# goroda/GPEXP

Measured on AMD Instinct MI355X. Metric: GP-fit+IVAR-eval points/s at N=32768 d=8 (wall-time in ms_per_step); value = (N+M)/t_step, SURVEY 8d's N/t_fit and M/t_IVAR are points_per_s_fit / points_per_s_ivar right behind it, higher is better.
Workload: dtype f64; 1 GPU; C4: N=32768 d=8 Matern-5/2 (rho=0.5,s=1,noise=0.1) kfill+potrf+potrs+logdet+IVAR over M=32768 MC points; N=32768, d=8, M=32768, kernel=matern52, seed=32768, parallelism=1 GPU

## Files before the change

gpexp_amd/_lib.py:

```python
import ctypes as C
import os

import numpy as np

_HERE = os.path.dirname(os.path.abspath(__file__))
LIB_PATH = os.path.join(_HERE, "libgpx_hip.so")

c_i64 = C.c_int64
c_dp = C.POINTER(C.c_double)
c_ip = C.POINTER(c_i64)
c_vp = C.c_void_p

_SIGS = {
    "gpx_abi_version": (C.c_int, []),
    "gpx_last_error": (C.c_char_p, []),
    "gpx_create": (C.c_int, [C.c_int, C.POINTER(c_vp)]),
    "gpx_destroy": (C.c_int, [c_vp]),
    "gpx_sync": (C.c_int, [c_vp]),
    "gpx_trim": (C.c_int, [c_vp]),
    "gpx_device_info": (C.c_int, [c_vp, C.c_char_p, C.c_int, C.POINTER(C.c_int), c_ip, C.POINTER(C.c_int)]),
    "gpx_mat_from_host": (C.c_int, [c_vp, c_dp, c_i64, c_i64, C.c_int, C.POINTER(c_vp)]),
    "gpx_mat_alloc": (C.c_int, [c_vp, c_i64, c_i64, C.c_int, C.POINTER(c_vp)]),
    "gpx_mat_free": (C.c_int, [c_vp, c_vp]),
    "gpx_mat_clone": (C.c_int, [c_vp, c_vp, C.POINTER(c_vp)]),
# ... 106 lines not shown
    "gpx_graph_free": (C.c_int, [c_vp, c_vp]),
    "gpx_dist2_unpack_rows": (C.c_int, [c_vp, c_vp, c_i64, c_i64, c_i64, c_i64, c_vp, c_i64, c_i64, c_i64]),
    "gpx_dist2_unpack_diag": (C.c_int, [c_vp, c_vp, c_i64, c_i64, c_i64, c_vp, c_i64]),
    "gpx_dist2_unpack_diag_at": (C.c_int, [c_vp, c_vp, c_i64, c_i64, c_i64, c_vp, c_i64, c_i64]),
    "gpx_dist2_trsv_diag": (C.c_int, [c_vp, c_vp, c_i64, c_i64, c_i64, c_vp, c_i64, C.c_int]),
    "gpx_dist2_gemv": (C.c_int, [c_vp, c_vp, c_i64, c_i64, c_i64, c_i64, c_vp, c_i64, c_vp, c_i64, C.c_int]),
    "gpx_dist2_logdet_acc": (C.c_int, [c_vp, c_vp, c_i64, c_i64, c_i64, c_i64, c_vp]),
    "gpx_stream_select": (C.c_int, [c_vp, C.c_int]),
    "gpx_event_record": (C.c_int, [c_vp, C.c_int]),
    "gpx_event_wait": (C.c_int, [c_vp, C.c_int]),
    "gpx_dist_finish": (C.c_int, [c_vp, c_vp]),
    "gpx_ivar_grad": (C.c_int, [c_vp, C.c_int, C.c_int, c_dp, C.c_int, c_vp, c_vp, c_vp, c_dp, c_dp]),
    "gpx_ivar_grad_w": (C.c_int, [c_vp, C.c_int, C.c_int, c_dp, C.c_int, c_vp, c_vp, c_vp, c_dp, c_vp, c_dp]),
    "gpx_ivar_grad_rows": (C.c_int, [c_vp, C.c_int, C.c_int, c_dp, C.c_int, c_vp, c_vp, c_vp, c_vp, c_i64, c_dp]),
    "gpx_var_grad": (C.c_int, [c_vp, C.c_int, C.c_int, c_dp, C.c_int, c_vp, c_vp, c_vp, c_dp, c_dp, c_dp, c_dp]),
    "gpx_var_grad_newpt": (C.c_int, [c_vp, C.c_int, C.c_int, c_dp, C.c_int, c_vp, c_vp, c_vp, c_dp]),
    "gpx_fitc_var_grad": (C.c_int, [c_vp, c_vp, C.c_int, C.c_int, c_dp, C.c_int, c_vp, c_vp, c_dp, c_dp, c_dp, c_dp]),
    "gpx_fitc_var_grad_newpt": (C.c_int, [c_vp, c_vp, C.c_int, C.c_int, c_dp, C.c_int, c_vp, c_vp, c_dp]),
    "gpx_profile_enable": (C.c_int, [c_vp, C.c_int]),
    "gpx_profile_reset": (C.c_int, [c_vp]),
    "gpx_profile_get": (C.c_int, [c_vp, C.c_int, c_ip, c_dp, c_dp, c_dp]),
    "gpx_dbg_gemm": (C.c_int, [c_vp, c_vp, c_vp, c_vp, C.c_int, C.c_int, C.c_int]),
    "gpx_dbg_gemm_strassen": (C.c_int, [c_vp, c_vp, c_vp, c_vp]),
    "gpx_dbg_gemm_tri": (C.c_int, [c_vp, c_vp, c_vp, c_vp, C.c_int, C.c_int, C.c_int]),
    "gpx_dbg_gemm_ksplit": (C.c_int, [c_vp, c_vp, c_vp, c_vp, C.c_int, C.c_int]),
    "gpx_dbg_kfill_plan": (C.c_int, [c_vp, C.c_int, C.c_int, c_dp, C.c_int, c_vp, c_vp, C.POINTER(C.c_int), c_dp]),
    "gpx_dbg_colreduce_plan": (C.c_int, [c_i64, c_i64, C.POINTER(c_i64), C.POINTER(c_i64)]),
    "gpx_dbg_panel_bcast_plan": (C.c_int, [C.c_int, C.c_int, c_i64, C.c_int, C.POINTER(c_i64), C.POINTER(C.c_int),
                                           C.POINTER(c_i64), c_i64, C.POINTER(c_i64)]),
    "gpx_dbg_guard_violations": (c_i64, [c_vp]),
    "gpx_dbg_guard_selftest": (C.c_int, [c_vp]),
    "gpx_dbg_spin": (C.c_int, [c_vp, C.c_int]),
    "gpx_dbg_spin_us": (C.c_int, [c_vp, c_i64]),
    "gpx_dbg_stamp": (C.c_int, [c_vp, C.c_int]),
    "gpx_dbg_spin_until": (C.c_int, [c_vp, C.c_int, c_i64]),
    "gpx_dbg_event_elapsed": (C.c_int, [c_vp, C.c_int, C.c_int, c_dp]),
    "gpx_dbg_leaf_stamps": (C.c_int, [c_vp, c_vp, C.c_int, C.POINTER(c_i64)]),
}

_lib = None


def load():
    global _lib
    if _lib is not None:
        return _lib
# ... 51 lines not shown
```

gpexp_amd/csrc/api.hip:

```cpp
#include "gpx_internal.h"
#include <stdarg.h>
#include <stdio.h>
#include <string.h>
#include <math.h>
#include <stdlib.h>

static thread_local char g_err[1024] = "";

void gpx_set_error(const char* fmt, ...) {
  va_list ap;
  va_start(ap, fmt);
  vsnprintf(g_err, sizeof(g_err), fmt, ap);
  va_end(ap);
}

static constexpr int64_t GUARD = 4096;

int gpx_dev_alloc(gpx_ctx* ctx, int64_t bytes, void** out) {
  if (bytes <= 0) bytes = 8;
  bytes = gpx_round_up(bytes, 256);
  const int64_t key = bytes + (ctx->guard ? 2 * GUARD : 0);
  void* base = nullptr;
  auto it = ctx->pool.find(key);
  if (it != ctx->pool.end()) {
// ... 1397 lines not shown
  GPX_TRY(gpx_dev_alloc(ctx, pb, &P));
  int r = mode <= 1 ? launch_gemm_ksplit(ctx, A->p, A->ld, B->p, B->ld, C->p, C->ld, m, n, k, mode == 1, parts, (double*)P)
                    : launch_gemm_ksplit_small(ctx, A->p, A->ld, B->p, B->ld, C->p, C->ld, m, n, k, mode == 3, parts, (double*)P);
  (void)hipStreamSynchronize(ctx->stream);
  gpx_dev_release(ctx, P, pb);
  return r;
}

int gpx_dbg_gemm(gpx_ctx* ctx, const gpx_mat* A, const gpx_mat* B, gpx_mat* C, int bt, int accumulate, int lower) {
  GPX_ARG(ctx && A && B && C, "NULL argument");
  const int64_t m = C->prows, n = C->pcols, k = A->pcols;
  GPX_ARG(A->prows == m, "A rows");
  GPX_ARG(bt ? (B->prows == n && B->pcols == k) : (B->prows == k && B->pcols == n), "B shape");
  GPX_TRY(launch_gemm(ctx, A->p, A->ld, B->p, B->ld, C->p, C->ld, m, n, k, bt != 0, accumulate != 0,
                      lower != 0));
  GPX_HIP(hipStreamSynchronize(ctx->stream));
  return 0;
}

int gpx_dbg_gemm_strassen(gpx_ctx* ctx, const gpx_mat* A, const gpx_mat* B, gpx_mat* C) {
  GPX_ARG(ctx && A && B && C, "NULL argument");
  const int64_t m = C->prows, n = C->pcols, k = A->pcols;
  GPX_ARG(A->prows == m && B->prows == k && B->pcols == n, "operand shapes");
  GPX_TRY(launch_gemm_strassen(ctx, A->p, A->ld, B->p, B->ld, C->p, C->ld, m, n, k, nullptr, 0));
  GPX_HIP(hipStreamSynchronize(ctx->stream));
  return 0;
}

}
```

gpexp_amd/csrc/chol.hip:

```cpp
#include "gpx_internal.h"
#include <math.h>
#include <stdlib.h>
#include <stddef.h>

namespace {

constexpr int NB = GPX_TILE;
constexpr int LS = NB + 1;

typedef double d4 __attribute__((ext_vector_type(4)));

__device__ __forceinline__ double readlane_d(double v, int srclane) {
  int lo = __builtin_amdgcn_readlane(__double2loint(v), srclane);
  int hi = __builtin_amdgcn_readlane(__double2hiint(v), srclane);
  return __hiloint2double(hi, lo);
}

constexpr int LB = 16;
constexpr int TS17 = LB + 1;
constexpr int BSZ = LB * TS17;
constexpr int LEAF_CB = LB * LB + 64 + LB;

__device__ __forceinline__ constexpr int sb_off(int I, int J) { return (I * (I + 1) / 2 + J) * BSZ; }

// ... 1176 lines not shown
  if (!Lm->binv) {
    void* p;
    GPX_TRY(gpx_dev_alloc(ctx, bytes, &p));
    Lm->binv = (double*)p;
    Lm->binv_bytes = bytes;
  }
  void* pt;
  GPX_TRY(gpx_dev_alloc(ctx, nblk * ib * ib * 8, &pt));
  int r = binv_build_range(ctx, Lm->p, Lm->ld, Lm->aux, Lm->binv, ib, n, (double*)pt);
  if (r == 0) r = chol_binv_finish(ctx, Lm, ib);
  (void)hipStreamSynchronize(ctx->stream);
  gpx_dev_release(ctx, pt, nblk * ib * ib * 8);
  if (r != 0) Lm->binv_ib = 0;
  return r;
}

struct PotrsPlan {
  const double* L;
  int64_t ld, n, ib, nblk;
  int64_t sib;
  const double* binv;
  const double* binvT;
  double* part;
  bool strassen = false;
  double* sscr = nullptr;
  int64_t sscr_bytes = 0;
};
static inline int64_t blk_off(const PotrsPlan& P, int64_t b) { return b * P.ib < P.n ? b * P.ib : P.n; }
static inline const double* blk_inv(const PotrsPlan& P, const double* base, int64_t b) {
  const int64_t row = b * P.ib, sb = row / P.sib, within = row - sb * P.sib;
  return base + sb * P.sib * P.sib + within * P.sib + within;
}

static int potrs_fwd(gpx_ctx* ctx, const PotrsPlan& P, int64_t b0, int64_t b1, double* rhs, double* x) {
  if (b1 - b0 == 1) {
    const int64_t o = blk_off(P, b0), sz = blk_off(P, b0 + 1) - o;
    hipLaunchKernelGGL(binv_gemv_kernel, dim3((unsigned)((sz + 3) / 4)), dim3(256), 0, ctx->stream, blk_inv(P, P.binv, b0),
                       P.sib, sz, rhs + o, x + o, 1);
    return 0;
  }
  const int64_t mid = (b0 + b1) / 2;
  GPX_TRY(potrs_fwd(ctx, P, b0, mid, rhs, x));
  const int64_t r0 = blk_off(P, mid), r1 = blk_off(P, b1), c0 = blk_off(P, b0);
  int64_t wg = (r1 - r0 + 3) / 4;
  if (wg > 4096) wg = 4096;
  hipLaunchKernelGGL(gemv_sub_kernel, dim3((unsigned)wg), dim3(256), 0, ctx->stream, P.L + r0 * P.ld + c0, P.ld, r1 - r0, r0 - c0,
                     x + c0, rhs + r0);
  return potrs_fwd(ctx, P, mid, b1, rhs, x);
}

static int potrs_bwd(gpx_ctx* ctx, const PotrsPlan& P, int64_t b0, int64_t b1, double* rhs, double* z) {
  if (b1 - b0 == 1) {
    const int64_t o = blk_off(P, b0), sz = blk_off(P, b0 + 1) - o;
    hipLaunchKernelGGL(binv_gemv_kernel, dim3((unsigned)((sz + 3) / 4)), dim3(256), 0, ctx->stream, blk_inv(P, P.binvT, b0),
                       P.sib, sz, rhs + o, z + o, 0);
    return 0;
  }
  const int64_t mid = (b0 + b1) / 2;
  GPX_TRY(potrs_bwd(ctx, P, mid, b1, rhs, z));
  const int64_t r0 = blk_off(P, mid), r1 = blk_off(P, b1), c0 = blk_off(P, b0);
  GPX_TRY(launch_colreduce(ctx, P.L + r0 * P.ld + c0, P.ld, r1 - r0, r0 - c0, z + r0, rhs + c0, P.part, 1));
  return potrs_bwd(ctx, P, b0, mid, rhs, z);
}

#ifndef GPX_STRASSEN_MIN_ROWS
#define GPX_STRASSEN_MIN_ROWS 8192
#endif
#ifndef GPX_STRASSEN_MIN_COLS
#define GPX_STRASSEN_MIN_COLS 4096
#endif
static inline bool strassen_gate(int64_t rows, int64_t cols, int64_t k) {
  return rows >= GPX_STRASSEN_MIN_ROWS && k >= GPX_STRASSEN_MIN_ROWS && cols >= GPX_STRASSEN_MIN_COLS &&
         gemm_strassen_scratch_bytes(rows, cols, k) > 0;
}

static int trsm_left_oop_rec(gpx_ctx* ctx, const PotrsPlan& P, int64_t b0, int64_t b1, double* B, int64_t ldb, double* W,
                             int64_t ldw, int64_t m) {
  if (b1 - b0 == 1) {
    const int64_t o = blk_off(P, b0), sz = blk_off(P, b0 + 1) - o;
    return launch_gemm_tri(ctx, blk_inv(P, P.binv, b0), P.sib, B + o * ldb, ldb, W + o * ldw, ldw, sz, m, sz, false, false,
                           false, 1);
  }
  const int64_t mid = (b0 + b1) / 2;
  GPX_TRY(trsm_left_oop_rec(ctx, P, b0, mid, B, ldb, W, ldw, m));
  const int64_t r0 = blk_off(P, mid), r1 = blk_off(P, b1), c0 = blk_off(P, b0);
  if (P.strassen && strassen_gate(r1 - r0, m, r0 - c0))
    GPX_TRY(launch_gemm_strassen(ctx, P.L + r0 * P.ld + c0, P.ld, W + c0 * ldw, ldw, B + r0 * ldb, ldb, r1 - r0, m, r0 - c0,
                                 P.sscr, P.sscr_bytes));
  else
    GPX_TRY(launch_gemm(ctx, P.L + r0 * P.ld + c0, P.ld, W + c0 * ldw, ldw, B + r0 * ldb, ldb, r1 - r0, m, r0 - c0, false,
                        true, false));
  return trsm_left_oop_rec(ctx, P, mid, b1, B, ldb, W, ldw, m);
}

int chol_trsm_left_oop(gpx_ctx* ctx, gpx_mat* Lm, double* B, int64_t ldb, double* W, int64_t ldw, int64_t m) {
  GPX_ARG(Lm && Lm->factored && Lm->aux && B && W && B != W, "trsm: matrix has not been factored / bad buffers");
  if (m == 0) return 0;
  GPX_TRY(chol_binv_ensure(ctx, Lm));
  PotrsPlan P;
  P.L = Lm->p;
  P.ld = Lm->ld;
  P.n = Lm->prows;
  P.sib = Lm->binv_ib;
  P.ib = P.sib < 1024 ? P.sib : 1024;
  P.nblk = (P.n + P.ib - 1) / P.ib;
  P.binv = Lm->binv;
  P.binvT = nullptr;
  P.part = nullptr;
  void* ps = nullptr;
  int64_t sbytes = 0;
  if (P.nblk >= 2 && env_i64("GPX_STRASSEN", 1) != 0) {
    const int64_t r0 = blk_off(P, P.nblk / 2);
    if (strassen_gate(P.n - r0, m, r0)) {
      sbytes = gemm_strassen_scratch_bytes(P.n - r0, m, r0);
      if (gpx_dev_alloc(ctx, sbytes, &ps) != 0) {
        (void)hipGetLastError();
        ps = nullptr;
      }
    }
  }
  P.strassen = ps != nullptr;
  P.sscr = (double*)ps;
  P.sscr_bytes = sbytes;
  const int r = trsm_left_oop_rec(ctx, P, 0, P.nblk, B, ldb, W, ldw, m);
  if (ps) {
    (void)hipStreamSynchronize(ctx->stream);
    gpx_dev_release(ctx, ps, sbytes);
  }
  return r;
}

int chol_trsm_left_group(gpx_ctx* ctx, const double* Lg, int64_t ld, const double* invd, int64_t w, int64_t below, int64_t ib,
                         double* B, int64_t ldb, int64_t m, double* inv, double* tmp, double* W, int64_t ldw) {
  GPX_ARG(Lg && invd && B && inv && tmp && W && W != B && w > 0 && w % NB == 0 && ib >= NB && ib % NB == 0, "trsm group: bad arguments");
  if (m == 0) return 0;
  GPX_TRY(binv_build_range(ctx, Lg, ld, invd, inv, ib, w, tmp));
  PotrsPlan P;
  P.L = Lg;
  P.ld = ld;
  P.n = w;
  P.ib = P.sib = ib;
  P.nblk = (w + ib - 1) / ib;
  P.binv = inv;
  P.binvT = nullptr;
// ... 71 lines not shown
```

gpexp_amd/csrc/gemm_f64.hip:

```cpp
#include "gpx_internal.h"
#include <stdlib.h>

namespace {

typedef double d4 __attribute__((ext_vector_type(4)));

constexpr int KB = 16;
constexpr int SA = KB + 1;

template <bool BT, int TE>
struct Smem {
  double a[2][TE * SA];
  double b[2][BT ? TE * SA : KB * (TE + 16)];
};

template <bool LOWER>
__device__ __forceinline__ bool tile_of(int sblk, int within, int tiles_m, int tiles_n, int sb_cols, int sb_shift,
                                        int* by, int* bx, int rot = 0) {
  const int sbm = (1 << sb_shift) - 1;
  int sr, sc;
  if (LOWER) {
    const int nsr = (tiles_m + sbm) >> sb_shift;
    const int noff = nsr * (nsr - 1) / 2;
    if (sblk < noff) {
// ... 19 lines not shown
  if (!LOWER && rot == 2) {
    *by = (sr << sb_shift) + (within & sbm);
    *bx = (sc << sb_shift) + (sbm - (within >> sb_shift));
  }
  if (!LOWER && rot == 4) {
    *by = (sr << sb_shift) + (sbm - (within >> sb_shift));
    *bx = (sc << sb_shift) + (within & sbm);
  }
  if (!LOWER && rot == 3) {
    *by = (sr << sb_shift) + (within & sbm);
    *bx = (sc << sb_shift) + (within >> sb_shift);
  }
  if (*by >= tiles_m || *bx >= tiles_n) return false;
  if (LOWER && *bx > *by) return false;
  return true;
}

struct NoSeg {
  static constexpr bool on = false;
};

struct NoDual {
  static constexpr bool on = false;
};
struct Dual {
  static constexpr bool on = true;
  double* c2;
  double s;
};

template <bool BT, bool ACC, int TE, class SEGF = NoSeg, class EPI = NoDual>
__device__ __forceinline__ void gemm_tile(Smem<BT, TE>& sm, const double* A, int64_t lda, const double* B, int64_t ldb,
                                          double* C, int64_t ldc, int nk, int by, int bx, const SEGF& segf = SEGF(),
                                          const EPI& epi = EPI()) {
  constexpr int SBN = TE + 16;
  constexpr int FI = TE / 32;
  constexpr int NL = TE / 32;
  constexpr int WS = TE / 2;
  constexpr int BKR = 512 / TE;
  constexpr int A_BUF = TE * SA;
  constexpr int B_BUF = BT ? TE * SA : KB * SBN;

  const int t = threadIdx.x;
  const int lane = t & 63, wave = t >> 6;
  const int wm = wave >> 1, wn = wave & 1;
  const int64_t m0 = (int64_t)by * TE, n0 = (int64_t)bx * TE;

  const int ar = t >> 3, ac = (t & 7) * 2;
  const int br = t / (TE / 2), bc = (t % (TE / 2)) * 2;
  const unsigned voff_a = (unsigned)((ar * lda + ac) * 8);
  const unsigned voff_b = BT ? (unsigned)((ar * ldb + ac) * 8) : (unsigned)((br * ldb + bc) * 8);
// ... 166 lines not shown
      GPX_MFMAS(3);
      GPX_FRAGS(buf ^ 1, 3, 3);
    }
    }
    GPX_MFMAS(0);
    GPX_MFMAS(1);
    GPX_MFMAS(2);
    GPX_MFMAS(3);
#undef GPX_STEP
#undef GPX_FRAGS
#undef GPX_MFMAS
#undef GPX_PIN
#undef GPX_PIN_ALL
  }
#undef GPX_GLOAD
#undef GPX_GLOAD_AT
#undef GPX_LD16
#undef GPX_SSTORE
#undef GPX_ST2
#undef GPX_STB
#undef GPX_COMPUTE

  double* Cw = C + (m0 + wm * WS + fk) * ldc + n0 + wn * WS + fr;
  if constexpr (EPI::on) {
    static_assert(ACC, "the two-destination epilogue accumulates");
    double* Cw2 = epi.c2 + (m0 + wm * WS + fk) * ldc + n0 + wn * WS + fr;
    const double s2 = epi.s;
#pragma unroll
    for (int i = 0; i < FI; ++i)
#pragma unroll
      for (int v = 0; v < 4; ++v) {
        double* cp = Cw + (int64_t)(i * 16 + 4 * v) * ldc;
        double* cq = Cw2 + (int64_t)(i * 16 + 4 * v) * ldc;
        double cv[FI], cw[FI];
#pragma unroll
        for (int j = 0; j < FI; ++j) {
          cv[j] = cp[j * 16];
          cw[j] = cq[j * 16];
        }
#pragma unroll
        for (int j = 0; j < FI; ++j) {
          cp[j * 16] = cv[j] - acc[i][j][v];
          cq[j * 16] = cw[j] - s2 * acc[i][j][v];
        }
      }
    return;
  }
// ... 49 lines not shown
    B += k0;
    nkt = nk - by * (TE / KB);
  }
  if (tri == 4) {
    const int64_t k0 = (int64_t)bx * TE;
    A += k0;
    B += k0 * ldb;
    nkt = nk - bx * (TE / KB);
  }
  gemm_tile<BT, ACC, TE>(sm, A, lda, B, ldb, C, ldc, nkt, by, bx);
}

template <int TE>
__global__ __launch_bounds__(256, 2) void gemm_f64_dual_kernel(const double* A, int64_t lda, const double* B, int64_t ldb,
                                                               double* C, double* C2, double s, int64_t ldc, int nk,
                                                               int tiles_m, int tiles_n, int sb_cols, int sb_shift) {
  __shared__ Smem<false, TE> sm;
  const int w = blockIdx.x;
  const int xcd = w & 7, q = w >> 3;
  const int sbs2 = 2 * sb_shift;
  int by, bx;
  if (!tile_of<false>((q >> sbs2) * 8 + xcd, q & ((1 << sbs2) - 1), tiles_m, tiles_n, sb_cols, sb_shift, &by, &bx, 0)) return;
  gemm_tile<false, true, TE, NoSeg, Dual>(sm, A, lda, B, ldb, C, ldc, nk, by, bx, NoSeg(), Dual{C2, s});
}

template <bool BSIDE>
__global__ __launch_bounds__(256) void strassen_sums_kernel(const double* __restrict__ X, int64_t ldx, int64_t hr, int64_t hc,
                                                            double* __restrict__ S, int64_t lds, int64_t sstride) {
  const int64_t j = ((int64_t)blockIdx.x * 256 + threadIdx.x) * 2;
  if (j >= hc) return;
  for (int64_t i = blockIdx.y; i < hr; i += gridDim.y) {
    const double* x1 = X + i * ldx + j;
    const double* x2 = X + (i + hr) * ldx + j;
    const double2 x11 = *reinterpret_cast<const double2*>(x1);
    const double2 x12 = *reinterpret_cast<const double2*>(x1 + hc);
    const double2 x21 = *reinterpret_cast<const double2*>(x2);
    const double2 x22 = *reinterpret_cast<const double2*>(x2 + hc);
    double* o = S + i * lds + j;
#define GPX_S2(k_, ex_, ey_) *reinterpret_cast<double2*>(o + (k_) * sstride) = make_double2(ex_, ey_)
    GPX_S2(0, x11.x + x22.x, x11.y + x22.y);
    if (BSIDE) {
      GPX_S2(1, x12.x - x22.x, x12.y - x22.y);
      GPX_S2(2, x21.x - x11.x, x21.y - x11.y);
      GPX_S2(3, x11.x + x12.x, x11.y + x12.y);
      GPX_S2(4, x21.x + x22.x, x21.y + x22.y);
    } else {
// ... 295 lines not shown
  return 0;
}

static int launch_gemm_dual(gpx_ctx* ctx, const double* A, int64_t lda, const double* B, int64_t ldb, double* C1, double* C2,
                            double s, int64_t ldc, int64_t m, int64_t n, int64_t k) {
  GPX_ARG(m % 128 == 0 && n % 128 == 0 && k % KB == 0 && k > 0 && m > 0 && n > 0, "gemm: m,n must be multiples of 128 and k of 16");
  GPX_ARG((lda % 2) == 0 && (ldb % 2) == 0, "gemm: leading dimensions must be even (16-byte loads)");
  const double tiles128 = (double)(m / 128) * (double)(n / 128);
  const int te = tiles128 < 1024.0 ? 64 : 128;
  const Plan p = make_plan(m, n, false, te);
  GPX_ARG(p.wgs < ((int64_t)1 << 31), "gemm: grid too large");
  const int nk = (int)(k / KB);
  ProfScope ps(ctx, GPX_PROF_GEMM, 2.0 * (double)m * (double)n * (double)k, 0.0);
  if (te == 64)
    hipLaunchKernelGGL(gemm_f64_dual_kernel<64>, dim3((unsigned)p.wgs), dim3(256), 0, ctx->stream, A, lda, B, ldb, C1, C2, s, ldc,
                       nk, p.tm, p.tn, p.sbc, p.sb_shift);
  else
    hipLaunchKernelGGL(gemm_f64_dual_kernel<128>, dim3((unsigned)p.wgs), dim3(256), 0, ctx->stream, A, lda, B, ldb, C1, C2, s, ldc,
                       nk, p.tm, p.tn, p.sbc, p.sb_shift);
  GPX_HIP(hipGetLastError());
  return 0;
}

static inline bool strassen_shape_ok(int64_t m, int64_t n, int64_t k) {
  return m > 0 && n > 0 && k > 0 && m % 256 == 0 && n % 256 == 0 && k % 32 == 0;
}

int64_t gemm_strassen_scratch_bytes(int64_t m, int64_t n, int64_t k) {
  if (!strassen_shape_ok(m, n, k)) return 0;
  const int64_t hm = m / 2, hn = n / 2, hk = k / 2;
  return 5 * (hm * gpx_skew_ld(hk) + hk * gpx_skew_ld(hn)) * 8;
}

int launch_gemm_strassen(gpx_ctx* ctx, const double* A, int64_t lda, const double* B, int64_t ldb, double* C, int64_t ldc,
                         int64_t m, int64_t n, int64_t k, double* scratch, int64_t scratch_bytes) {
  const int64_t need = gemm_strassen_scratch_bytes(m, n, k);
  if (need == 0 || (lda % 2) != 0 || (ldb % 2) != 0 || C == A || C == B)
    return launch_gemm(ctx, A, lda, B, ldb, C, ldc, m, n, k, false, true, false);
  void* own = nullptr;
  if (!scratch || scratch_bytes < need) {
    if (gpx_dev_alloc(ctx, need, &own) != 0) {
      (void)hipGetLastError();
      return launch_gemm(ctx, A, lda, B, ldb, C, ldc, m, n, k, false, true, false);
    }
    scratch = (double*)own;
  }
  const int64_t hm = m / 2, hn = n / 2, hk = k / 2, lsa = gpx_skew_ld(hk), lsb = gpx_skew_ld(hn);
  const int64_t sa = hm * lsa, sb = hk * lsb;
  double* const S = scratch;
  double* const T = scratch + 5 * sa;
  int r = 0;
  do {
    {
      ProfScope ps(ctx, GPX_PROF_REDUCE, 5.0 * (double)hm * hk + 5.0 * (double)hk * hn, 72.0 * ((double)hm * hk + (double)hk * hn));
      hipLaunchKernelGGL(strassen_sums_kernel<false>, dim3((unsigned)((hk / 2 + 255) / 256), (unsigned)(hm < 65535 ? hm : 65535)),
                         dim3(256), 0, ctx->stream, A, lda, hm, hk, S, lsa, sa);
      hipLaunchKernelGGL(strassen_sums_kernel<true>, dim3((unsigned)((hn / 2 + 255) / 256), (unsigned)(hk < 65535 ? hk : 65535)),
                         dim3(256), 0, ctx->stream, B, ldb, hk, hn, T, lsb, sb);
      if (hipGetLastError() != hipSuccess) {
        gpx_set_error("strassen: operand-sum launch failed");
        r = -2;
        break;
      }
    }
    const double *A11 = A, *A22 = A + hm * lda + hk, *B11 = B, *B22 = B + hk * ldb + hn;
    double *C11 = C, *C12 = C + hn, *C21 = C + hm * ldc, *C22 = C + hm * ldc + hn;
    if ((r = launch_gemm_dual(ctx, S, lsa, T, lsb, C11, C22, 1.0, ldc, hm, hn, hk)) != 0) break;
    if ((r = launch_gemm_dual(ctx, S + sa, lsa, B11, ldb, C21, C22, -1.0, ldc, hm, hn, hk)) != 0) break;
    if ((r = launch_gemm_dual(ctx, A11, lda, T + sb, lsb, C12, C22, 1.0, ldc, hm, hn, hk)) != 0) break;
    if ((r = launch_gemm_dual(ctx, A22, lda, T + 2 * sb, lsb, C11, C21, 1.0, ldc, hm, hn, hk)) != 0) break;
    if ((r = launch_gemm_dual(ctx, S + 2 * sa, lsa, B22, ldb, C12, C11, -1.0, ldc, hm, hn, hk)) != 0) break;
    if ((r = launch_gemm(ctx, S + 3 * sa, lsa, T + 3 * sb, lsb, C22, ldc, hm, hn, hk, false, true, false)) != 0) break;
    if ((r = launch_gemm(ctx, S + 4 * sa, lsa, T + 4 * sb, lsb, C11, ldc, hm, hn, hk, false, true, false)) != 0) break;
  } while (0);
  if (own) {
    (void)hipStreamSynchronize(ctx->stream);
    gpx_dev_release(ctx, own, need);
  }
  return r;
}

int launch_dist2_update(gpx_ctx* ctx, double* C, int64_t ldc, int64_t lr0, int64_t m, int64_t lc0, int64_t n, int64_t nb, int Pr,
                        int Pc, int pr, int pc, int64_t piece_stride, int64_t dsz, int nseg, const double* const* g,
                        const int64_t* ks, int below_diag) {
  if (m == 0 || n == 0 || nseg == 0) return 0;
  GPX_ARG(nseg > 0 && nseg <= GPX_SEG_MAX && Pr >= 1 && Pr <= GPX_MAX_PR && Pc >= 1, "dist2 update: too many segments / grid rows");
  GPX_ARG(m % 128 == 0 && n % 128 == 0 && nb % 128 == 0 && lr0 % nb == 0 && lc0 % nb == 0 && (ldc % 2) == 0, "dist2 update: alignment");
  Dist2Upd u;
  for (int s = 0; s < nseg; ++s) {
    u.g[s] = g[s];
    for (int p = 0; p < Pr; ++p) u.li0[s][p] = (int)(ks[s] + 1 <= p ? 0 : (ks[s] - p) / Pr + 1);
  }
  u.nseg = nseg;
  u.seg_nk = (int)(nb / KB);
  u.Pr = Pr; u.Pc = Pc; u.pr = pr; u.pc = pc;
  u.nb = (int)nb;
  u.gld = (int)gpx_g_ld(nb);
// ... 66 lines not shown
```

gpexp_amd/csrc/gpx_internal.h:

```cpp
#pragma once
#include <hip/hip_runtime.h>
#include <stdint.h>
#include <stdlib.h>
#include <string>
#include <vector>
#include <map>
#include <memory>
#include <unordered_set>
#include "../../include/gpx.h"
#include "../../include/gpx_dist.h"
#include "../../include/gpx_debug.h"

#define GPX_TILE 128
#define GPX_MAXD GPX_MAX_DIM
#define GPX_NSTREAMS 6
#define GPX_SEG_MAX 8
#ifndef GPX_G_SKEW
#define GPX_G_SKEW 0
#endif
#define GPX_MAX_PR 4

void gpx_set_error(const char* fmt, ...);
#define GPX_HIP(call)                                                                   \
  do {                                                                                  \
// ... 138 lines not shown

int launch_kfill(gpx_ctx* ctx, const KParams& kp, const double* A, int64_t na, const double* B, int64_t nb,
                 int symmetric, const double* d_nugget, int64_t nugget_len, double nugget_scalar,
                 double* out, int64_t prows, int64_t pcols, int64_t ld);
int launch_kfill_offset(gpx_ctx* ctx, const KParams& kp, const double* X, int64_t n, int64_t row_off, int64_t col_off,
                        const double* d_nugget, int64_t nugget_len, double nugget_scalar, double* out, int64_t prows,
                        int64_t pcols, int64_t ld);
int launch_kdiag(gpx_ctx* ctx, const KParams& kp, const double* Z, int64_t m, double* out);
int launch_kfill_cyclic(gpx_ctx* ctx, const KParams& kp, const double* X, int64_t n, const double* d_nugget,
                        int64_t nugget_len, double nugget_scalar, double* out, int64_t prows, int64_t pcols, int64_t ld,
                        int64_t nb, int Pr, int pr, int Pc, int pc);
int gpx_copy2d(gpx_ctx* ctx, const double* src, int64_t lds_, double* dst, int64_t ldd, int64_t rows, int64_t cols);
int gpx_copy2d_lower(gpx_ctx* ctx, const double* src, int64_t lds_, double* dst, int64_t ldd, int64_t n);
int launch_kfill_rows(gpx_ctx* ctx, const KParams& kp, const double* X, int64_t n, int64_t row0, const double* d_nugget,
                      int64_t nugget_len, double nugget_scalar, double* out, int64_t prows_band, int64_t pcols,
                      int64_t ld);

static inline int gpx_chain_prio(const gpx_ctx* ctx) { return ctx->stream == ctx->streams[1] ? 1 : 0; }
int launch_gemm(gpx_ctx* ctx, const double* A, int64_t lda, const double* B, int64_t ldb, double* C, int64_t ldc,
                int64_t m, int64_t n, int64_t k, bool bt, bool accumulate, bool lower);

int launch_gemm_tri(gpx_ctx* ctx, const double* A, int64_t lda, const double* B, int64_t ldb, double* C, int64_t ldc,
                    int64_t m, int64_t n, int64_t k, bool bt, bool accumulate, bool lower, int tri);
int64_t gemm_strassen_scratch_bytes(int64_t m, int64_t n, int64_t k);
int launch_gemm_strassen(gpx_ctx* ctx, const double* A, int64_t lda, const double* B, int64_t ldb, double* C, int64_t ldc,
                         int64_t m, int64_t n, int64_t k, double* scratch, int64_t scratch_bytes);
int launch_gemm_ksplit(gpx_ctx* ctx, const double* A, int64_t lda, const double* B, int64_t ldb, double* C, int64_t ldc,
                       int64_t m, int64_t n, int64_t k, bool lower, int64_t parts, double* P, bool assign = false);
int launch_gemm_ksplit_small(gpx_ctx* ctx, const double* A, int64_t lda, const double* B, int64_t ldb, double* C, int64_t ldc,
                             int64_t m, int64_t n, int64_t k, bool assign, int64_t parts, double* P);
int launch_gemm_batched(gpx_ctx* ctx, const double* A, int64_t lda, int64_t sa, const double* B, int64_t ldb, int64_t sb,
                        double* C, int64_t ldc, int64_t sc, int64_t m, int64_t n, int64_t k, bool bt, bool accumulate,
                        int64_t batch);

int launch_dist2_update(gpx_ctx* ctx, double* C, int64_t ldc, int64_t lr0, int64_t m, int64_t lc0, int64_t n, int64_t nb, int Pr,
                        int Pc, int pr, int pc, int64_t piece_stride, int64_t dsz, int nseg, const double* const* g,
                        const int64_t* ks, int below_diag);

int launch_leaf(gpx_ctx* ctx, double* A, int64_t ld, double* inv, int64_t base_index, int64_t n_valid);
int chol_potrf(gpx_ctx* ctx, double* A, int64_t ld, int64_t n, double* invd, int64_t n_valid);
int chol_potrf_nozero(gpx_ctx* ctx, double* A, int64_t ld, int64_t n, double* invd, int64_t base, int64_t n_valid);
int chol_trsm_right(gpx_ctx* ctx, const double* L, int64_t ldl, const double* invd, double* X, int64_t ldx,
                    int64_t m, int64_t n);
int chol_trsm_right_n(gpx_ctx* ctx, const double* L, int64_t ldl, const double* invd, double* X, int64_t ldx,
                      int64_t m, int64_t n);
int chol_trsm_left(gpx_ctx* ctx, const double* L, int64_t ldl, const double* invd, double* B, int64_t ldb,
                   int64_t n, int64_t m);
int chol_trsv(gpx_ctx* ctx, const double* L, int64_t ld, const double* invd, double* y, int64_t n, bool transposed);
int64_t chol_trsv_scratch_bytes(int64_t n);
// ... 38 lines not shown
```

gpexp_amd/device.py:

```python
import ctypes as C
import atexit
import os

import numpy as np

from . import _lib
from ._lib import check, as_f64, dptr, c_vp, c_i64, GpxError

K_SE, K_MATERN32, K_MATERN52, K_MEHLER = 0, 1, 2, 3
PROF_CLASSES = ["kfill", "gemm", "leaf", "trsv", "reduce", "greedy", "comm", "kcross"]

_ctx = None


class Context:

    def __init__(self, device=None):
        self.lib = _lib.load()
        if device is None:
            device = int(os.environ.get("LOCAL_RANK", "0"))
        h = c_vp()
        rc = self.lib.gpx_create(int(device), C.byref(h))
        if rc != 0:
            raise RuntimeError("gpexp_amd needs an MI355X: " + self.lib.gpx_last_error().decode())
# ... 631 lines not shown


def kfill_plan(ctx, spec, X, Z=None):
    ex = C.c_int()
    cen = np.zeros(spec.d)
    check(ctx.lib.gpx_dbg_kfill_plan(ctx.h, *spec.args(), X.h, Z.h if Z is not None else None, C.byref(ex), dptr(cen)))
    return bool(ex.value), cen


def dbg_gemm_tri(ctx, A, B, Cm, bt, accumulate, tri):
    check(ctx.lib.gpx_dbg_gemm_tri(ctx.h, A.h, B.h, Cm.h, int(bt), int(accumulate), int(tri)))


def dbg_gemm_ksplit(ctx, A, B, Cm, mode, parts):
    check(ctx.lib.gpx_dbg_gemm_ksplit(ctx.h, A.h, B.h, Cm.h, int(mode), int(parts)))


def dbg_gemm(ctx, A, B, Cm, bt, accumulate, lower=False):
    check(ctx.lib.gpx_dbg_gemm(ctx.h, A.h, B.h, Cm.h, int(bt), int(accumulate), int(lower)))


def dbg_gemm_strassen(ctx, A, B, Cm):
    check(ctx.lib.gpx_dbg_gemm_strassen(ctx.h, A.h, B.h, Cm.h))
```

include/gpx_debug.h:

```cpp
#ifndef GPX_DEBUG_H
#define GPX_DEBUG_H
#include "gpx.h"
#ifdef __cplusplus
extern "C" {
#endif

int gpx_dbg_gemm(gpx_ctx* ctx, const gpx_mat* A, const gpx_mat* B, gpx_mat* C, int bt, int accumulate, int lower);
int gpx_dbg_gemm_tri(gpx_ctx* ctx, const gpx_mat* A, const gpx_mat* B, gpx_mat* C, int bt, int accumulate, int tri);
int gpx_dbg_gemm_ksplit(gpx_ctx* ctx, const gpx_mat* A, const gpx_mat* B, gpx_mat* C, int mode, int parts);
int gpx_dbg_gemm_strassen(gpx_ctx* ctx, const gpx_mat* A, const gpx_mat* B, gpx_mat* C);
int gpx_dbg_spin(gpx_ctx* ctx, int ms);
int64_t gpx_dbg_guard_violations(gpx_ctx* ctx);
int gpx_dbg_guard_selftest(gpx_ctx* ctx);
int gpx_dbg_panel_bcast_plan(int W, int me, int64_t small_elems, int npieces, const int64_t* counts, const int* roots,
                             int64_t* ops, int64_t max_ops, int64_t* nops);
int gpx_dbg_colreduce_plan(int64_t rows, int64_t pcols, int64_t* nchunk, int64_t* bound_elems);
int gpx_dbg_kfill_plan(gpx_ctx* ctx, int kind, int d, const double* hyp, int nhyp, const gpx_mat* X, const gpx_mat* Z,
                       int* exact, double* center);

int gpx_dbg_spin_us(gpx_ctx* ctx, int64_t us);
int gpx_dbg_stamp(gpx_ctx* ctx, int slot);
int gpx_dbg_spin_until(gpx_ctx* ctx, int slot, int64_t us);
int gpx_dbg_event_elapsed(gpx_ctx* ctx, int id0, int id1, double* ms);

int gpx_dbg_leaf_stamps(gpx_ctx* ctx, gpx_mat* K, int fast, int64_t* out30);

#ifdef __cplusplus
}
#endif
#endif
```

Measured before the change: 102,700 points/s.

## Generalise Strassen GEMM to two recursion levels with multi-destination epilogue

Replaces the hard-coded one-level Strassen used in the blocked triangular solve with a recursive scheme of up to two levels. A new GEMM kernel writes one product into several scaled destinations, so the leaf products of depth-2 Strassen are accumulated directly. The gate picks depth 2 when all operand dimensions are at least 16384, and scratch is allocated for the chosen depth, falling back to shallower depth if allocation fails. Depth 2 cuts f64 MFMA work further but adds operand-sum kernels, more scratch memory, epilogues that touch up to four output tiles, and extra rounding error.

```diff
diff --git a/gpexp_amd/_lib.py b/gpexp_amd/_lib.py
--- a/gpexp_amd/_lib.py
+++ b/gpexp_amd/_lib.py
@@ -152,6 +152,7 @@
     "gpx_profile_get": (C.c_int, [c_vp, C.c_int, c_ip, c_dp, c_dp, c_dp]),
     "gpx_dbg_gemm": (C.c_int, [c_vp, c_vp, c_vp, c_vp, C.c_int, C.c_int, C.c_int]),
     "gpx_dbg_gemm_strassen": (C.c_int, [c_vp, c_vp, c_vp, c_vp]),
+    "gpx_dbg_gemm_strassen_depth": (C.c_int, [c_vp, c_vp, c_vp, c_vp, C.c_int]),
     "gpx_dbg_gemm_tri": (C.c_int, [c_vp, c_vp, c_vp, c_vp, C.c_int, C.c_int, C.c_int]),
     "gpx_dbg_gemm_ksplit": (C.c_int, [c_vp, c_vp, c_vp, c_vp, C.c_int, C.c_int]),
     "gpx_dbg_kfill_plan": (C.c_int, [c_vp, C.c_int, C.c_int, c_dp, C.c_int, c_vp, c_vp, C.POINTER(C.c_int), c_dp]),
diff --git a/gpexp_amd/csrc/api.hip b/gpexp_amd/csrc/api.hip
--- a/gpexp_amd/csrc/api.hip
+++ b/gpexp_amd/csrc/api.hip
@@ -1443,9 +1443,19 @@
   GPX_ARG(ctx && A && B && C, "NULL argument");
   const int64_t m = C->prows, n = C->pcols, k = A->pcols;
   GPX_ARG(A->prows == m && B->prows == k && B->pcols == n, "operand shapes");
-  GPX_TRY(launch_gemm_strassen(ctx, A->p, A->ld, B->p, B->ld, C->p, C->ld, m, n, k, nullptr, 0));
+  GPX_TRY(launch_gemm_strassen(ctx, A->p, A->ld, B->p, B->ld, C->p, C->ld, m, n, k, 1, nullptr, 0));
   GPX_HIP(hipStreamSynchronize(ctx->stream));
   return 0;
 }
 
-}
+int gpx_dbg_gemm_strassen_depth(gpx_ctx* ctx, const gpx_mat* A, const gpx_mat* B, gpx_mat* C, int depth) {
+  GPX_ARG(ctx && A && B && C, "NULL argument");
+  GPX_ARG(depth >= 0 && depth <= GPX_STRASSEN_MAX_DEPTH, "strassen: depth out of range");
+  const int64_t m = C->prows, n = C->pcols, k = A->pcols;
+  GPX_ARG(A->prows == m && B->prows == k && B->pcols == n, "operand shapes");
+  GPX_TRY(launch_gemm_strassen(ctx, A->p, A->ld, B->p, B->ld, C->p, C->ld, m, n, k, depth, nullptr, 0));
+  GPX_HIP(hipStreamSynchronize(ctx->stream));
+  return 0;
+}
+
+}
diff --git a/gpexp_amd/csrc/chol.hip b/gpexp_amd/csrc/chol.hip
--- a/gpexp_amd/csrc/chol.hip
+++ b/gpexp_amd/csrc/chol.hip
@@ -1,4 +1,5 @@
 #include "gpx_internal.h"
+#include <algorithm>
 #include <math.h>
 #include <stdlib.h>
 #include <stddef.h>
@@ -1222,7 +1223,7 @@
   const double* binv;
   const double* binvT;
   double* part;
-  bool strassen = false;
+  int strassen = 0;
   double* sscr = nullptr;
   int64_t sscr_bytes = 0;
 };
@@ -1269,9 +1270,20 @@
 #ifndef GPX_STRASSEN_MIN_COLS
 #define GPX_STRASSEN_MIN_COLS 4096
 #endif
-static inline bool strassen_gate(int64_t rows, int64_t cols, int64_t k) {
-  return rows >= GPX_STRASSEN_MIN_ROWS && k >= GPX_STRASSEN_MIN_ROWS && cols >= GPX_STRASSEN_MIN_COLS &&
-         gemm_strassen_scratch_bytes(rows, cols, k) > 0;
+#ifndef GPX_STRASSEN2_MIN_ROWS
+#define GPX_STRASSEN2_MIN_ROWS 16384
+#endif
+#ifndef GPX_STRASSEN2_MIN_COLS
+#define GPX_STRASSEN2_MIN_COLS 16384
+#endif
+static inline int strassen_gate(int64_t rows, int64_t cols, int64_t k) {
+  if (!(rows >= GPX_STRASSEN_MIN_ROWS && k >= GPX_STRASSEN_MIN_ROWS && cols >= GPX_STRASSEN_MIN_COLS &&
+        gemm_strassen_scratch_bytes(rows, cols, k, 1) > 0))
+    return 0;
+  if (!(rows >= GPX_STRASSEN2_MIN_ROWS && k >= GPX_STRASSEN2_MIN_ROWS && cols >= GPX_STRASSEN2_MIN_COLS &&
+        gemm_strassen_scratch_bytes(rows, cols, k, 2) > 0))
+    return 1;
+  return 2;
 }
 
 static int trsm_left_oop_rec(gpx_ctx* ctx, const PotrsPlan& P, int64_t b0, int64_t b1, double* B, int64_t ldb, double* W,
@@ -1284,9 +1296,10 @@
   const int64_t mid = (b0 + b1) / 2;
   GPX_TRY(trsm_left_oop_rec(ctx, P, b0, mid, B, ldb, W, ldw, m));
   const int64_t r0 = blk_off(P, mid), r1 = blk_off(P, b1), c0 = blk_off(P, b0);
-  if (P.strassen && strassen_gate(r1 - r0, m, r0 - c0))
+  const int depth = P.strassen ? std::min(P.strassen, strassen_gate(r1 - r0, m, r0 - c0)) : 0;
+  if (depth > 0)
     GPX_TRY(launch_gemm_strassen(ctx, P.L + r0 * P.ld + c0, P.ld, W + c0 * ldw, ldw, B + r0 * ldb, ldb, r1 - r0, m, r0 - c0,
-                                 P.sscr, P.sscr_bytes));
+                                 depth, P.sscr, P.sscr_bytes));
   else
     GPX_TRY(launch_gemm(ctx, P.L + r0 * P.ld + c0, P.ld, W + c0 * ldw, ldw, B + r0 * ldb, ldb, r1 - r0, m, r0 - c0, false,
                         true, false));
@@ -1309,17 +1322,18 @@
   P.part = nullptr;
   void* ps = nullptr;
   int64_t sbytes = 0;
-  if (P.nblk >= 2 && env_i64("GPX_STRASSEN", 1) != 0) {
+  int depth = 0;
+  const int64_t max_depth = env_i64("GPX_STRASSEN", GPX_STRASSEN_MAX_DEPTH);
+  if (P.nblk >= 2 && max_depth > 0) {
     const int64_t r0 = blk_off(P, P.nblk / 2);
-    if (strassen_gate(P.n - r0, m, r0)) {
-      sbytes = gemm_strassen_scratch_bytes(P.n - r0, m, r0);
-      if (gpx_dev_alloc(ctx, sbytes, &ps) != 0) {
-        (void)hipGetLastError();
-        ps = nullptr;
-      }
-    }
-  }
-  P.strassen = ps != nullptr;
+    for (depth = (int)std::min<int64_t>(max_depth, strassen_gate(P.n - r0, m, r0)); depth > 0; --depth) {
+      sbytes = gemm_strassen_scratch_bytes(P.n - r0, m, r0, depth);
+      if (sbytes > 0 && gpx_dev_alloc(ctx, sbytes, &ps) == 0) break;
+      (void)hipGetLastError();
+      ps = nullptr;
+    }
+  }
+  P.strassen = ps ? depth : 0;
   P.sscr = (double*)ps;
   P.sscr_bytes = sbytes;
   const int r = trsm_left_oop_rec(ctx, P, 0, P.nblk, B, ldb, W, ldw, m);
diff --git a/gpexp_amd/csrc/gemm_f64.hip b/gpexp_amd/csrc/gemm_f64.hip
--- a/gpexp_amd/csrc/gemm_f64.hip
+++ b/gpexp_amd/csrc/gemm_f64.hip
@@ -65,11 +65,20 @@
 
 struct NoDual {
   static constexpr bool on = false;
+  static constexpr bool multi = false;
 };
 struct Dual {
   static constexpr bool on = true;
+  static constexpr bool multi = false;
   double* c2;
   double s;
+};
+constexpr int GPX_MULTI_MAX = 1 << GPX_STRASSEN_MAX_DEPTH;
+struct Multi {
+  static constexpr bool multi = true;
+  double* c[GPX_MULTI_MAX];
+  double s[GPX_MULTI_MAX];
+  int nd;
 };
 
 template <bool BT, bool ACC, int TE, class SEGF = NoSeg, class EPI = NoDual>
@@ -282,7 +291,28 @@
 #undef GPX_COMPUTE
 
   double* Cw = C + (m0 + wm * WS + fk) * ldc + n0 + wn * WS + fr;
-  if constexpr (EPI::on) {
+  if constexpr (EPI::multi) {
+    static_assert(ACC, "the multi-destination epilogue accumulates");
+    const int64_t coff = (m0 + wm * WS + fk) * ldc + n0 + wn * WS + fr;
+#pragma unroll
+    for (int d = 0; d < GPX_MULTI_MAX; ++d) {
+      if (d >= epi.nd) break;
+      double* const Cd = epi.c[d] + coff;
+      const double sd = epi.s[d];
+#pragma unroll
+      for (int i = 0; i < FI; ++i)
+#pragma unroll
+        for (int v = 0; v < 4; ++v) {
+          double* cp = Cd + (int64_t)(i * 16 + 4 * v) * ldc;
+          double cv[FI];
+#pragma unroll
+          for (int j = 0; j < FI; ++j) cv[j] = cp[j * 16];
+#pragma unroll
+          for (int j = 0; j < FI; ++j) cp[j * 16] = cv[j] - sd * acc[i][j][v];
+        }
+    }
+    return;
+  } else if constexpr (EPI::on) {
     static_assert(ACC, "the two-destination epilogue accumulates");
     double* Cw2 = epi.c2 + (m0 + wm * WS + fk) * ldc + n0 + wn * WS + fr;
     const double s2 = epi.s;
@@ -378,6 +408,19 @@
   int by, bx;
   if (!tile_of<false>((q >> sbs2) * 8 + xcd, q & ((1 << sbs2) - 1), tiles_m, tiles_n, sb_cols, sb_shift, &by, &bx, 0)) return;
   gemm_tile<false, true, TE, NoSeg, Dual>(sm, A, lda, B, ldb, C, ldc, nk, by, bx, NoSeg(), Dual{C2, s});
+}
+
+template <int TE>
+__global__ __launch_bounds__(256, 2) void gemm_f64_multi_kernel(const double* A, int64_t lda, const double* B, int64_t ldb,
+                                                                const Multi dst, int64_t ldc, int nk, int tiles_m, int tiles_n,
+                                                                int sb_cols, int sb_shift) {
+  __shared__ Smem<false, TE> sm;
+  const int w = blockIdx.x;
+  const int xcd = w & 7, q = w >> 3;
+  const int sbs2 = 2 * sb_shift;
+  int by, bx;
+  if (!tile_of<false>((q >> sbs2) * 8 + xcd, q & ((1 << sbs2) - 1), tiles_m, tiles_n, sb_cols, sb_shift, &by, &bx, 0)) return;
+  gemm_tile<false, true, TE, NoSeg, Multi>(sm, A, lda, B, ldb, dst.c[0], ldc, nk, by, bx, NoSeg(), dst);
 }
 
 template <bool BSIDE>
@@ -719,57 +762,134 @@
   return 0;
 }
 
-static inline bool strassen_shape_ok(int64_t m, int64_t n, int64_t k) {
-  return m > 0 && n > 0 && k > 0 && m % 256 == 0 && n % 256 == 0 && k % 32 == 0;
-}
-
-int64_t gemm_strassen_scratch_bytes(int64_t m, int64_t n, int64_t k) {
-  if (!strassen_shape_ok(m, n, k)) return 0;
-  const int64_t hm = m / 2, hn = n / 2, hk = k / 2;
-  return 5 * (hm * gpx_skew_ld(hk) + hk * gpx_skew_ld(hn)) * 8;
-}
-
-int launch_gemm_strassen(gpx_ctx* ctx, const double* A, int64_t lda, const double* B, int64_t ldb, double* C, int64_t ldc,
-                         int64_t m, int64_t n, int64_t k, double* scratch, int64_t scratch_bytes) {
-  const int64_t need = gemm_strassen_scratch_bytes(m, n, k);
-  if (need == 0 || (lda % 2) != 0 || (ldb % 2) != 0 || C == A || C == B)
-    return launch_gemm(ctx, A, lda, B, ldb, C, ldc, m, n, k, false, true, false);
-  void* own = nullptr;
-  if (!scratch || scratch_bytes < need) {
-    if (gpx_dev_alloc(ctx, need, &own) != 0) {
-      (void)hipGetLastError();
-      return launch_gemm(ctx, A, lda, B, ldb, C, ldc, m, n, k, false, true, false);
-    }
-    scratch = (double*)own;
+static int launch_gemm_multi(gpx_ctx* ctx, const double* A, int64_t lda, const double* B, int64_t ldb, const Multi& dst,
+                             int64_t ldc, int64_t m, int64_t n, int64_t k) {
+  GPX_ARG(m % 128 == 0 && n % 128 == 0 && k % KB == 0 && k > 0 && m > 0 && n > 0, "gemm: m,n must be multiples of 128 and k of 16");
+  GPX_ARG((lda % 2) == 0 && (ldb % 2) == 0, "gemm: leading dimensions must be even (16-byte loads)");
+  GPX_ARG(dst.nd >= 1 && dst.nd <= GPX_MULTI_MAX, "gemm: bad destination count");
+  const double tiles128 = (double)(m / 128) * (double)(n / 128);
+  const int te = tiles128 < 1024.0 ? 64 : 128;
+  const Plan p = make_plan(m, n, false, te);
+  GPX_ARG(p.wgs < ((int64_t)1 << 31), "gemm: grid too large");
+  const int nk = (int)(k / KB);
+  ProfScope ps(ctx, GPX_PROF_GEMM, 2.0 * (double)m * (double)n * (double)k, 0.0);
+  if (te == 64)
+    hipLaunchKernelGGL(gemm_f64_multi_kernel<64>, dim3((unsigned)p.wgs), dim3(256), 0, ctx->stream, A, lda, B, ldb, dst, ldc, nk,
+                       p.tm, p.tn, p.sbc, p.sb_shift);
+  else
+    hipLaunchKernelGGL(gemm_f64_multi_kernel<128>, dim3((unsigned)p.wgs), dim3(256), 0, ctx->stream, A, lda, B, ldb, dst, ldc, nk,
+                       p.tm, p.tn, p.sbc, p.sb_shift);
+  GPX_HIP(hipGetLastError());
+  return 0;
+}
+
+static inline bool strassen_shape_ok(int64_t m, int64_t n, int64_t k, int depth) {
+  return depth >= 1 && depth <= GPX_STRASSEN_MAX_DEPTH && m > 0 && n > 0 && k > 0 && m % ((int64_t)128 << depth) == 0 &&
+         n % ((int64_t)128 << depth) == 0 && k % ((int64_t)KB << depth) == 0;
+}
+
+static inline int64_t strassen_level_elems(int64_t hm, int64_t hn, int64_t hk) {
+  return 5 * (hm * gpx_skew_ld(hk) + hk * gpx_skew_ld(hn));
+}
+
+int64_t gemm_strassen_scratch_bytes(int64_t m, int64_t n, int64_t k, int depth) {
+  if (!strassen_shape_ok(m, n, k, depth)) return 0;
+  int64_t elems = 0;
+  for (int d = 0; d < depth; ++d) {
+    m /= 2, n /= 2, k /= 2;
+    elems += strassen_level_elems(m, n, k);
+  }
+  return elems * 8;
+}
+
+namespace {
+struct SDest {
+  double* c;
+  double s;
+};
+struct SProd {
+  int a, b, nq, q[2];
+  double s[2];
+};
+constexpr SProd kStrassen[7] = {
+    {-1, -1, 2, {0, 3}, {1.0, 1.0}},
+    {-2, 0, 2, {2, 3}, {1.0, -1.0}},
+    {0, -2, 2, {1, 3}, {1.0, 1.0}},
+    {3, -3, 2, {0, 2}, {1.0, 1.0}},
+    {-3, 3, 2, {1, 0}, {1.0, -1.0}},
+    {-4, -4, 1, {3, 0}, {1.0, 0.0}},
+    {-5, -5, 1, {0, 0}, {1.0, 0.0}},
+};
+}
+
+static int strassen_rec(gpx_ctx* ctx, const double* A, int64_t lda, const double* B, int64_t ldb, const SDest* dst, int nd,
+                        int64_t ldc, int64_t m, int64_t n, int64_t k, int depth, double* scratch) {
+  if (depth == 0) {
+    for (int d = 1; d < nd; ++d)
+      for (int e = 0; e < d; ++e) GPX_ARG(dst[d].c != dst[e].c, "strassen: two destinations of one product coincide");
+    if (nd == 1 && dst[0].s == 1.0) return launch_gemm(ctx, A, lda, B, ldb, dst[0].c, ldc, m, n, k, false, true, false);
+    if (nd == 2 && dst[0].s == 1.0) return launch_gemm_dual(ctx, A, lda, B, ldb, dst[0].c, dst[1].c, dst[1].s, ldc, m, n, k);
+    GPX_ARG(nd >= 1 && nd <= GPX_MULTI_MAX, "strassen: too many destinations for one product");
+    Multi md;
+    for (int d = 0; d < GPX_MULTI_MAX; ++d) {
+      md.c[d] = d < nd ? dst[d].c : nullptr;
+      md.s[d] = d < nd ? dst[d].s : 0.0;
+    }
+    md.nd = nd;
+    return launch_gemm_multi(ctx, A, lda, B, ldb, md, ldc, m, n, k);
   }
   const int64_t hm = m / 2, hn = n / 2, hk = k / 2, lsa = gpx_skew_ld(hk), lsb = gpx_skew_ld(hn);
   const int64_t sa = hm * lsa, sb = hk * lsb;
   double* const S = scratch;
   double* const T = scratch + 5 * sa;
-  int r = 0;
-  do {
-    {
-      ProfScope ps(ctx, GPX_PROF_REDUCE, 5.0 * (double)hm * hk + 5.0 * (double)hk * hn, 72.0 * ((double)hm * hk + (double)hk * hn));
-      hipLaunchKernelGGL(strassen_sums_kernel<false>, dim3((unsigned)((hk / 2 + 255) / 256), (unsigned)(hm < 65535 ? hm : 65535)),
-                         dim3(256), 0, ctx->stream, A, lda, hm, hk, S, lsa, sa);
-      hipLaunchKernelGGL(strassen_sums_kernel<true>, dim3((unsigned)((hn / 2 + 255) / 256), (unsigned)(hk < 65535 ? hk : 65535)),
-                         dim3(256), 0, ctx->stream, B, ldb, hk, hn, T, lsb, sb);
-      if (hipGetLastError() != hipSuccess) {
-        gpx_set_error("strassen: operand-sum launch failed");
-        r = -2;
-        break;
+  double* const below = T + 5 * sb;
+  {
+    ProfScope ps(ctx, GPX_PROF_REDUCE, 5.0 * (double)hm * hk + 5.0 * (double)hk * hn, 72.0 * ((double)hm * hk + (double)hk * hn));
+    hipLaunchKernelGGL(strassen_sums_kernel<false>, dim3((unsigned)((hk / 2 + 255) / 256), (unsigned)(hm < 65535 ? hm : 65535)),
+                       dim3(256), 0, ctx->stream, A, lda, hm, hk, S, lsa, sa);
+    hipLaunchKernelGGL(strassen_sums_kernel<true>, dim3((unsigned)((hn / 2 + 255) / 256), (unsigned)(hk < 65535 ? hk : 65535)),
+                       dim3(256), 0, ctx->stream, B, ldb, hk, hn, T, lsb, sb);
+    if (hipGetLastError() != hipSuccess) {
+      gpx_set_error("strassen: operand-sum launch failed");
+      return -2;
+    }
+  }
+  const int64_t qoff[4] = {0, hn, hm * ldc, hm * ldc + hn};
+  for (const SProd& p : kStrassen) {
+    const double* Ap = p.a < 0 ? S + (-1 - p.a) * sa : (p.a == 0 ? A : A + hm * lda + hk);
+    const double* Bp = p.b < 0 ? T + (-1 - p.b) * sb : (p.b == 0 ? B : B + hk * ldb + hn);
+    SDest sub[GPX_MULTI_MAX];
+    int ns = 0;
+    for (int d = 0; d < nd; ++d)
+      for (int j = 0; j < p.nq; ++j) {
+        GPX_ARG(ns < GPX_MULTI_MAX, "strassen: too many destinations for one product");
+        sub[ns++] = SDest{dst[d].c + qoff[p.q[j]], dst[d].s * p.s[j]};
       }
-    }
-    const double *A11 = A, *A22 = A + hm * lda + hk, *B11 = B, *B22 = B + hk * ldb + hn;
-    double *C11 = C, *C12 = C + hn, *C21 = C + hm * ldc, *C22 = C + hm * ldc + hn;
-    if ((r = launch_gemm_dual(ctx, S, lsa, T, lsb, C11, C22, 1.0, ldc, hm, hn, hk)) != 0) break;
-    if ((r = launch_gemm_dual(ctx, S + sa, lsa, B11, ldb, C21, C22, -1.0, ldc, hm, hn, hk)) != 0) break;
-    if ((r = launch_gemm_dual(ctx, A11, lda, T + sb, lsb, C12, C22, 1.0, ldc, hm, hn, hk)) != 0) break;
-    if ((r = launch_gemm_dual(ctx, A22, lda, T + 2 * sb, lsb, C11, C21, 1.0, ldc, hm, hn, hk)) != 0) break;
-    if ((r = launch_gemm_dual(ctx, S + 2 * sa, lsa, B22, ldb, C12, C11, -1.0, ldc, hm, hn, hk)) != 0) break;
-    if ((r = launch_gemm(ctx, S + 3 * sa, lsa, T + 3 * sb, lsb, C22, ldc, hm, hn, hk, false, true, false)) != 0) break;
-    if ((r = launch_gemm(ctx, S + 4 * sa, lsa, T + 4 * sb, lsb, C11, ldc, hm, hn, hk, false, true, false)) != 0) break;
-  } while (0);
+    GPX_TRY(strassen_rec(ctx, Ap, p.a < 0 ? lsa : lda, Bp, p.b < 0 ? lsb : ldb, sub, ns, ldc, hm, hn, hk, depth - 1, below));
+  }
+  return 0;
+}
+
+int launch_gemm_strassen(gpx_ctx* ctx, const double* A, int64_t lda, const double* B, int64_t ldb, double* C, int64_t ldc,
+                         int64_t m, int64_t n, int64_t k, int depth, double* scratch, int64_t scratch_bytes) {
+  if (depth > GPX_STRASSEN_MAX_DEPTH) depth = GPX_STRASSEN_MAX_DEPTH;
+  if ((lda % 2) != 0 || (ldb % 2) != 0 || C == A || C == B) depth = 0;
+  void* own = nullptr;
+  int64_t need = 0;
+  for (; depth > 0; --depth) {
+    need = gemm_strassen_scratch_bytes(m, n, k, depth);
+    if (need == 0) continue;
+    if (scratch && scratch_bytes >= need) break;
+    if (gpx_dev_alloc(ctx, need, &own) == 0) {
+      scratch = (double*)own;
+      break;
+    }
+    (void)hipGetLastError();
+    own = nullptr;
+  }
+  if (depth <= 0) return launch_gemm(ctx, A, lda, B, ldb, C, ldc, m, n, k, false, true, false);
+  const SDest top{C, 1.0};
+  const int r = strassen_rec(ctx, A, lda, B, ldb, &top, 1, ldc, m, n, k, depth, scratch);
   if (own) {
     (void)hipStreamSynchronize(ctx->stream);
     gpx_dev_release(ctx, own, need);
diff --git a/gpexp_amd/csrc/gpx_internal.h b/gpexp_amd/csrc/gpx_internal.h
--- a/gpexp_amd/csrc/gpx_internal.h
+++ b/gpexp_amd/csrc/gpx_internal.h
@@ -184,9 +184,10 @@
 
 int launch_gemm_tri(gpx_ctx* ctx, const double* A, int64_t lda, const double* B, int64_t ldb, double* C, int64_t ldc,
                     int64_t m, int64_t n, int64_t k, bool bt, bool accumulate, bool lower, int tri);
-int64_t gemm_strassen_scratch_bytes(int64_t m, int64_t n, int64_t k);
+constexpr int GPX_STRASSEN_MAX_DEPTH = 2;
+int64_t gemm_strassen_scratch_bytes(int64_t m, int64_t n, int64_t k, int depth);
 int launch_gemm_strassen(gpx_ctx* ctx, const double* A, int64_t lda, const double* B, int64_t ldb, double* C, int64_t ldc,
-                         int64_t m, int64_t n, int64_t k, double* scratch, int64_t scratch_bytes);
+                         int64_t m, int64_t n, int64_t k, int depth, double* scratch, int64_t scratch_bytes);
 int launch_gemm_ksplit(gpx_ctx* ctx, const double* A, int64_t lda, const double* B, int64_t ldb, double* C, int64_t ldc,
                        int64_t m, int64_t n, int64_t k, bool lower, int64_t parts, double* P, bool assign = false);
 int launch_gemm_ksplit_small(gpx_ctx* ctx, const double* A, int64_t lda, const double* B, int64_t ldb, double* C, int64_t ldc,
diff --git a/gpexp_amd/device.py b/gpexp_amd/device.py
--- a/gpexp_amd/device.py
+++ b/gpexp_amd/device.py
@@ -677,3 +677,7 @@
 
 def dbg_gemm_strassen(ctx, A, B, Cm):
     check(ctx.lib.gpx_dbg_gemm_strassen(ctx.h, A.h, B.h, Cm.h))
+
+
+def dbg_gemm_strassen_depth(ctx, A, B, Cm, depth):
+    check(ctx.lib.gpx_dbg_gemm_strassen_depth(ctx.h, A.h, B.h, Cm.h, int(depth)))
diff --git a/include/gpx_debug.h b/include/gpx_debug.h
--- a/include/gpx_debug.h
+++ b/include/gpx_debug.h
@@ -9,6 +9,7 @@
 int gpx_dbg_gemm_tri(gpx_ctx* ctx, const gpx_mat* A, const gpx_mat* B, gpx_mat* C, int bt, int accumulate, int tri);
 int gpx_dbg_gemm_ksplit(gpx_ctx* ctx, const gpx_mat* A, const gpx_mat* B, gpx_mat* C, int mode, int parts);
 int gpx_dbg_gemm_strassen(gpx_ctx* ctx, const gpx_mat* A, const gpx_mat* B, gpx_mat* C);
+int gpx_dbg_gemm_strassen_depth(gpx_ctx* ctx, const gpx_mat* A, const gpx_mat* B, gpx_mat* C, int depth);
 int gpx_dbg_spin(gpx_ctx* ctx, int ms);
 int64_t gpx_dbg_guard_violations(gpx_ctx* ctx);
 int gpx_dbg_guard_selftest(gpx_ctx* ctx);
diff --git a/profiles/strassen2_isa_compare.py b/profiles/strassen2_isa_compare.py
--- /dev/null
+++ b/profiles/strassen2_isa_compare.py
@@ -0,0 +1,67 @@
+#!/usr/bin/env python3
+import re
+import sys
+
+
+def functions(path):
+    out, name, body = {}, None, []
+    for line in open(path):
+        m = re.match(r"^([A-Za-z_][\w$.]*):\s*(;.*)?$", line)
+        if m and not m.group(1).startswith(".L") and name is None:
+            name, body = m.group(1), []
+            continue
+        if name is not None:
+            if line.startswith(".Lfunc_end"):
+                out[name] = body
+                name = None
+                continue
+            t = line.split(";", 1)[0].strip()
+            if not t or t.startswith((".p2align", ".loc", ".cfi", ".file")):
+                continue
+            body.append(re.sub(r"\.LBB\d+_(\d+)", r".LBB_\1", t))
+    return out
+
+
+def k_loop(body):
+    blocks, cur = [], []
+    for t in body:
+        if t.startswith(".LBB_") and t.endswith(":"):
+            blocks.append(cur)
+            cur = []
+        else:
+            cur.append(t)
+    blocks.append(cur)
+    return max(blocks, key=lambda b: sum(1 for t in b if t.startswith("v_mfma")))
+
+
+def main():
+    a, b = functions(sys.argv[1]), functions(sys.argv[2])
+    bad = 0
+    for name in sorted(a):
+        if name not in b:
+            print("MISSING  ", name)
+            bad += 1
+        elif a[name] != b[name]:
+            print("DIFFERENT", name, len(a[name]), len(b[name]))
+            bad += 1
+    print("%d functions in the first file, %d identical in the second, %d new: %s"
+          % (len(a), len(a) - bad, len(set(b) - set(a)), " ".join(sorted(set(b) - set(a)))))
+    if "--loop" in sys.argv:
+        i = sys.argv.index("--loop")
+        new = [n for n in b if sys.argv[i + 1] in n]
+        ref = [n for n in b if sys.argv[i + 2] in n]
+        assert len(new) == 1 and len(ref) == 1, (new, ref)
+        ln, lr = k_loop(b[new[0]]), k_loop(b[ref[0]])
+        on, orr = [t.split()[0] for t in ln], [t.split()[0] for t in lr]
+        print("k-loop of %s: %d instructions, %d MFMAs; of %s: %d, %d; opcode for opcode: %s"
+              % (new[0], len(on), sum(o.startswith("v_mfma") for o in on), ref[0], len(orr),
+                 sum(o.startswith("v_mfma") for o in orr), "IDENTICAL" if on == orr else "DIFFERENT"))
+        for j in range(min(len(on), len(orr))):
+            if on[j] != orr[j]:
+                print("  position %d: %s   |   %s" % (j, ln[j], lr[j]))
+        bad += on != orr
+    return 1 if bad else 0
+
+
+if __name__ == "__main__":
+    sys.exit(main())
```

Result: faster. 105,100 points/s, median of 6 (+2.3%).
